# mahfuzalhasan/WaveFormer

Measured on AMD Instinct MI355X. Metric: 128³×4 volumes/sec fwd (1/2/4/8 MI355X) + Dice Δ vs reference, higher is better.
Workload: dtype bf16x3; 1 GPU; MultiscaleTransformer (WaveFormer encoder) forward, 128^3x4 crops; global_batch=8, per_gpu_batch=8, precision=bf16x3, parallelism=replicas x1 (no data-path collective), hip_graph=True

## Files before the change

### waveformer_amd/csrc/ffn_dwfc_tb.hip

```cpp
#include "kernels.hpp"

namespace wf {

#ifndef WF_TB_EPRIO
#define WF_TB_EPRIO 3
#endif

namespace tb4 {
constexpr int S2 = 4;
constexpr int C = 48, HID = 192, TY = 4, TX = 8;
constexpr int PY = TY + 2, PX = TX + 2, PP = PY * PX;
constexpr int NPOS = TY * TX;
constexpr int HS = HID + 8;
constexpr int PLANE_F = PP * HID;
constexpr int H2F = NPOS * HS;
constexpr int NV = HID / 4;
constexpr int NPC = (PP * NV + 63) / 64;
constexpr int NPCE = (NPC + 3) / 4;
constexpr int KS = HID / 32;
constexpr int FWL_BYTES = (C / 16) * KS * 64 * 16;
constexpr size_t LDS_BYTES = (size_t)(2 * PLANE_F + 2 * H2F + 2 * HID + 2 * C) * 4 + FWL_BYTES;
static_assert(LDS_BYTES <= 160 * 1024, "LDS");
}

template <int P>
__global__ __launch_bounds__(1024, 1) void ffn_dwfc_tb4_kernel(DwFcArgs a) {
  using namespace tb4;
  constexpr bool SPLIT = P == PREC_SPLIT;
  __shared__ __attribute__((aligned(16))) float planes[2 * PLANE_F];
  __shared__ __attribute__((aligned(16))) float h2b[2 * H2F];
  __shared__ __attribute__((aligned(16))) float vecs[2 * HID + 2 * C];
  __shared__ bf16x8 fwlo[FWL_BYTES / 16];
  float* lnw = vecs;
  float* lnb = lnw + HID;
  float* fcl = lnb + HID;
  float* n2w = fcl + C;
  __shared__ int simd_cnt[4];

  const int tid = threadIdx.x;
  const int wid = tid >> 6, lane = tid & 63;
  const int D = a.D, H = a.H, W = a.W;
  const int ntx = (W + TX - 1) / TX, nty = (H + TY - 1) / TY, nzs = (D + a.ZS - 1) / a.ZS;
  const int nb = gridDim.x;
  const int xcd = blockIdx.x & 7, q8 = nb >> 3, r8 = nb & 7;
  int t = (xcd < r8 ? xcd * (q8 + 1) : r8 * (q8 + 1) + (xcd - r8) * q8) + (blockIdx.x >> 3);
  const int xt = t % ntx;
  t /= ntx;
  const int yt = t % nty;
  t /= nty;
  const int zt = t % nzs;
  const int b = t / nzs;
  const int x0 = xt * TX, y0 = yt * TY, z0 = zt * a.ZS, z1 = min(z0 + a.ZS, D);
  const int64_t plane_sz = (int64_t)H * W;

  if (tid < 4) simd_cnt[tid] = 0;
  for (int i = tid; i < HID; i += 1024) {
    lnw[i] = 0.5f * a.ln2_w[i];
    lnb[i] = 0.5f * a.ln2_b[i];
  }
  for (int i = tid; i < C; i += 1024) {
    fcl[i] = (a.fc_b ? a.fc_b[i] : 0.f) + (a.stats ? a.n2_b[i] : 0.f);
    n2w[i] = a.stats ? a.n2_w[i] : 1.f;
  }
  if (SPLIT) {
    for (int i = tid; i < (C / 16) * KS * 64; i += 1024) {
      const int l = i & 63, ks = (i >> 6) % KS, ct = (i >> 6) / KS;
      fwlo[i] = *reinterpret_cast<const bf16x8*>(a.fc + (size_t)C * HID +
                                                 (size_t)(ct * 16 + (l & 15)) * HID + ks * 32 + 8 * (l >> 4));
    }
  }
  for (int i = tid; i < HID * 27; i += 1024) planes[i] = a.dw_w[i];
  for (int i = tid; i < HID; i += 1024) planes[HID * 27 + i] = a.dw_b[i];
  __syncthreads();
  const int simd = tb_simd_id();
  int slot = 0;
  if (lane == 0) slot = atomicAdd(&simd_cnt[simd], 1);
  slot = __builtin_amdgcn_readfirstlane(__shfl(slot, 0, 64));
  __syncthreads();
  const bool even = simd_cnt[0] == 4 && simd_cnt[1] == 4 && simd_cnt[2] == 4 && simd_cnt[3] == 4;
  int role = even ? (slot < 3 ? 3 * simd + slot : 12 + simd) : wid;
  role = __builtin_amdgcn_readfirstlane(role);

  if (role < 12) {
    const int cp = role / 3, kslot = role % 3, c = kslot * 64 + lane;
    float w[27];
#pragma unroll
    for (int k = 0; k < 27; ++k) w[k] = planes[c * 27 + k];
    const float bias = planes[HID * 27 + c];
    float acc[3][TY][2];
#pragma unroll
    for (int s = 0; s < 3; ++s)
#pragma unroll
      for (int o = 0; o < TY; ++o) acc[s][o][0] = acc[s][o][1] = 0.f;
    const int lpos = 8 * cp + 4 * kslot + (lane >> 4), lg = lane & 15;
    const int cm = 4 * ((lg - 2 * lpos) & 15);
    __syncthreads();
    __syncthreads();

    auto ln2_rows = [&](float* h2t) {
      constexpr int LNC = HID / 16;
      float* row = h2t + lpos * HS;
      float v[LNC];
#pragma unroll
      for (int j = 0; j < LNC / 4; ++j) {
        const f32x4 u = *reinterpret_cast<const f32x4*>(row + cm + 64 * j);
        v[4 * j] = u.x;
        v[4 * j + 1] = u.y;
        v[4 * j + 2] = u.z;
        v[4 * j + 3] = u.w;
      }
      float s4[4];
#pragma unroll
      for (int j = 0; j < 4; ++j) s4[j] = (v[j] + v[j + 4]) + v[j + 8];
      const float mean = group_sum<16>((s4[0] + s4[1]) + (s4[2] + s4[3])) * (1.f / HID);
      float q4[4];
#pragma unroll
      for (int j = 0; j < 4; ++j) {
        const float d0 = v[j] - mean, d1 = v[j + 4] - mean, d2 = v[j + 8] - mean;
        q4[j] = d2 * d2 + (d1 * d1 + d0 * d0);
      }
      const float rstd = __builtin_amdgcn_rsqf(
          group_sum<16>((q4[0] + q4[1]) + (q4[2] + q4[3])) * (1.f / HID) + a.eps2);
      const float nmr = -mean * rstd;
      uint16_t* rowh = reinterpret_cast<uint16_t*>(row);
#pragma unroll
      for (int j = 0; j < LNC / 4; ++j) {
        const int cc = cm + 64 * j;
        const f32x4 lw4 = *reinterpret_cast<const f32x4*>(lnw + cc);
        const f32x4 lb4 = *reinterpret_cast<const f32x4*>(lnb + cc);
        const f32x4 y = gelu_half4((f32x4{v[4 * j], v[4 * j + 1], v[4 * j + 2], v[4 * j + 3]} *
                                    rstd + nmr) * lw4 + lb4);
        uint32_t h0, h1, l0, l1;
        split_pair<P>(y[0], y[1], h0, l0);
        split_pair<P>(y[2], y[3], h1, l1);
        *reinterpret_cast<u32x2*>(rowh + cc) = u32x2{h0, h1};
        if (SPLIT) *reinterpret_cast<u32x2*>(rowh + HID + cc) = u32x2{l0, l1};
      }
    };
    auto rows = [&](const float (&vin)[PY][4], auto SAc, auto SBc, auto SCc, auto LOc, auto HIc) {
      constexpr int SA = decltype(SAc)::value, SB = decltype(SBc)::value,
                    SC = decltype(SCc)::value, LO = decltype(LOc)::value, HI = decltype(HIc)::value;
#pragma unroll
      for (int r = LO; r < HI; ++r) {
        const float* v = vin[r];
#pragma unroll
        for (int ky = 0; ky < 3; ++ky) {
          const int o = r - ky;
          if (o < 0 || o >= TY) continue;
          const float* w0 = w + ky * 3;
#pragma unroll
          for (int j = 0; j < 2; ++j) {
            if (ky == 0)
              acc[SC][o][j] = w0[2] * v[j + 2] + (w0[1] * v[j + 1] + w0[0] * v[j]);
            else
              acc[SC][o][j] = w0[2] * v[j + 2] + (w0[1] * v[j + 1] + (w0[0] * v[j] + acc[SC][o][j]));
            acc[SB][o][j] = w0[11] * v[j + 2] + (w0[10] * v[j + 1] + (w0[9] * v[j] + acc[SB][o][j]));
            acc[SA][o][j] = w0[20] * v[j + 2] + (w0[19] * v[j + 1] + (w0[18] * v[j] + acc[SA][o][j]));
          }
        }
      }
    };
    typedef std::integral_constant<int, 0> I0;
    typedef std::integral_constant<int, S2> IS;
    typedef std::integral_constant<int, PY> IP;
    auto step = [&](int p, auto Rc) {
      constexpr int R = decltype(Rc)::value;
      typedef std::integral_constant<int, R> SA;
      typedef std::integral_constant<int, (R + 1) % 3> SB;
      typedef std::integral_constant<int, (R + 2) % 3> SC;
      const bool live = p <= z1 && !(ffn_dbg(a) & 1);
      const bool ln = p - 2 >= z0 && p - 2 < z1 && !(ffn_dbg(a) & 2);
      float vin[PY][4];
      const float* q0 = planes + ((p - z0 + 1) & 1) * PLANE_F + 2 * cp * HID + c;
      auto load_plane = [&]() {
#pragma unroll
        for (int r = 0; r < PY; ++r)
#pragma unroll
          for (int k = 0; k < 4; ++k) vin[r][k] = q0[(r * PX + k) * HID];
      };
      if (kslot < 2) {
        if (ln) ln2_rows(h2b + ((p - 2 - z0) & 1) * H2F);
        if (live) load_plane();
      } else if (live) {
        load_plane();
        rows(vin, SA(), SB(), SC(), I0(), IS());
      }
      __syncthreads();
      if (live) {
        if (kslot < 2) rows(vin, SA(), SB(), SC(), I0(), IP());
        else rows(vin, SA(), SB(), SC(), IS(), IP());
        if (p - 1 >= z0) {
          float* h2t = h2b + ((p - 1 - z0) & 1) * H2F;
#pragma unroll
          for (int o = 0; o < TY; ++o)
#pragma unroll
            for (int j = 0; j < 2; ++j)
              h2t[(o * TX + 2 * cp + j) * HS + c] = acc[R][o][j] + bias;
        }
      }
      __syncthreads();
    };
    for (int p = z0 - 1; p <= z1 + 1; p += 3) {
      step(p, std::integral_constant<int, 0>());
      if (p + 1 <= z1 + 1) step(p + 1, std::integral_constant<int, 1>());
      if (p + 2 <= z1 + 1) step(p + 2, std::integral_constant<int, 2>());
    }
    return;
  }

  __builtin_amdgcn_s_setprio(WF_TB_EPRIO);
  const int e = role - 12;
  const int l15 = lane & 15, g4 = lane >> 4;
  const bool has_fc = e < C / 16;
  const int ct = has_fc ? e : 0;
  const float bs = a.bscale ? a.bscale[b] : 1.f;
  bf16x8 fwh[KS];
  {
    const uint16_t* wr = a.fc + (size_t)(ct * 16 + l15) * HID + 8 * g4;
#pragma unroll
    for (int ks = 0; ks < KS; ++ks) fwh[ks] = *reinterpret_cast<const bf16x8*>(wr + ks * 32);
  }
  const bf16x8* fwl = fwlo + ct * KS * 64 + lane;
  const float* src = reinterpret_cast<const float*>(a.h1) + (int64_t)b * D * H * W * HID;
  const int64_t plane_elems = (int64_t)H * W * HID;
  auto piece_off = [&](int k) {
    const int i = min((4 * k + e) * 64 + lane, PP * NV - 1);
    const int pos = i / NV, v = i - pos * NV;
    const int yy = y0 - 1 + pos / PX, xx = x0 - 1 + pos % PX;
    const bool ok = yy >= 0 && yy < H && xx >= 0 && xx < W;
    return ok ? (uint32_t)(((yy * W + xx) * HID + 4 * v) * 4) : 0x80000000u;
  };
  auto stage = [&](int p, float* dst) {
    const bool pz = p >= 0 && p < D;
    const float* base = src + (int64_t)min(max(p, 0), D - 1) * plane_elems;
    const __amdgpu_buffer_rsrc_t rs = __builtin_amdgcn_make_buffer_rsrc(
        const_cast<float*>(base), 0, pz ? (int)(plane_elems * 4) : 0, 0x00020000);
#pragma unroll
    for (int k = 0; k < NPCE; ++k) {
      const int j = 4 * k + e;
      const uint32_t o = piece_off(k);
      if (j * 64 < PP * NV && (j * 64 + lane < PP * NV))
        __builtin_amdgcn_raw_ptr_buffer_load_lds(
            rs, (__attribute__((address_space(3))) void*)(dst + j * 256), 16, o, 0, 0, 0);
    }
  };
  const int col = ct * 16 + 4 * g4;
  const float* sbase = a.stats ? a.stats : a.x;
  auto gpos_of = [&](int zo, int rt, bool clamp) {
    const int lp = rt * 16 + l15;
    int yo = y0 + lp / TX, xo = x0 + lp % TX;
    if (clamp) {
      yo = min(yo, H - 1);
      xo = min(xo, W - 1);
    }
    return (int64_t)b * D * plane_sz + (int64_t)zo * plane_sz + (int64_t)yo * W + xo;
  };
  auto row_ok = [&](int rt) {
    const int lp = rt * 16 + l15;
    return y0 + lp / TX < H && x0 + lp % TX < W;
  };
  f32x4 xr[2][2];
  f32x2 es[2][2];
  const int64_t npos = (int64_t)a.B * D * plane_sz;
  const __amdgpu_buffer_rsrc_t xrsrc = __builtin_amdgcn_make_buffer_rsrc(
      const_cast<float*>(a.x), 0, (int)(npos * C * 4), 0x00020000);
  const __amdgpu_buffer_rsrc_t srsrc = __builtin_amdgcn_make_buffer_rsrc(
      const_cast<float*>(sbase), 0, (int)(npos * 2 * 4), 0x00020000);
  auto load_resid = [&](int zo, f32x4 (&xv)[2], f32x2 (&ev)[2]) {
#pragma unroll
    for (int rt = 0; rt < 2; ++rt) {
      const int g = (int)gpos_of(zo, rt, true);
      xv[rt] = __builtin_bit_cast(f32x4, __builtin_amdgcn_raw_buffer_load_b128(xrsrc, (g * C + col) * 4, 0, 0));
      ev[rt] = __builtin_bit_cast(f32x2, __builtin_amdgcn_raw_buffer_load_b64(srsrc, g * 8, 0, 0));
    }
  };
  const __amdgpu_buffer_rsrc_t orsrc = __builtin_amdgcn_make_buffer_rsrc(
      a.out, 0, (int)(npos * C * 4), 0x00020000);
  auto fc_store = [&](const float* h2t, int zo, int rt, const f32x4& xv, const f32x2& ev) {
    const int lp = rt * 16 + l15;
    f32x4 acc = f32x4{0.f, 0.f, 0.f, 0.f};
    const uint16_t* Bh = reinterpret_cast<const uint16_t*>(h2t) + (size_t)lp * (2 * HS);
#pragma unroll
    for (int ks = 0; ks < KS; ++ks) {
      const int k = ks * 32 + 8 * g4;
      const bf16x8 bh = *reinterpret_cast<const bf16x8*>(Bh + k);
      if (SPLIT) {
        const bf16x8 bl = *reinterpret_cast<const bf16x8*>(Bh + HID + k);
        acc = mma32<P>(fwh[ks], bl, acc);
        acc = mma32<P>(fwl[ks * 64], bh, acc);
      }
      acc = mma32<P>(fwh[ks], bh, acc);
    }
    f32x4 v = acc + *reinterpret_cast<const f32x4*>(fcl + col);
    if (a.stats) {
      const f32x4 lw = *reinterpret_cast<const f32x4*>(n2w + col);
      v = xv + ((xv - ev.x) * ev.y * lw + v) * bs;
    } else {
      v = xv + v * bs;
    }
    const int voff = row_ok(rt) ? (int)((gpos_of(zo, rt, false) * C + col) * 4) : (int)0x80000000;
    __builtin_amdgcn_raw_buffer_store_b128(__builtin_bit_cast(u32x4, v), orsrc, voff, 0, 0);
  };

  __syncthreads();
  stage(z0 - 1, planes);
  asm volatile("s_waitcnt vmcnt(0)" ::: "memory");
  __syncthreads();
  auto iter = [&](int p, auto Sc) {
    constexpr int S = decltype(Sc)::value;
    const int zo = p - 2;
    const bool epi = has_fc && zo >= z0 && zo < z1;
    if (has_fc && zo + 1 >= z0 && zo + 1 < z1) load_resid(zo + 1, xr[S ^ 1], es[S ^ 1]);
    if (p + 1 <= z1 && !(ffn_dbg(a) & 8)) stage(p + 1, planes + ((p + 2 - z0) & 1) * PLANE_F);
    __builtin_amdgcn_s_barrier();
    if (epi && !(ffn_dbg(a) & 4)) {
      const float* h2t = h2b + ((zo - z0) & 1) * H2F;
      fc_store(h2t, zo, 0, xr[S][0], es[S][0]);
      fc_store(h2t, zo, 1, xr[S][1], es[S][1]);
      asm volatile("s_waitcnt vmcnt(2)" ::: "memory");
    } else {
      asm volatile("s_waitcnt vmcnt(0)" ::: "memory");
    }
    asm volatile("s_waitcnt lgkmcnt(0)" ::: "memory");
    __builtin_amdgcn_s_barrier();
  };
  for (int p = z0 - 1; p <= z1 + 1; p += 2) {
    iter(p, std::integral_constant<int, 1>());
    if (p + 1 <= z1 + 1) iter(p + 1, std::integral_constant<int, 0>());
  }
}

int launch_ffn_dwfc_tb4(const DwFcArgs& a, int prec, hipStream_t s) {
  using namespace tb4;
  DwFcArgs g = a;
  static int cus = 0;
  if (!cus) {
    int dev = 0;
    (void)hipGetDevice(&dev);
    (void)hipDeviceGetAttribute(&cus, hipDeviceAttributeMultiprocessorCount, dev);
    if (cus <= 0) cus = 256;
  }
  const int64_t base = (int64_t)g.B * cdiv(g.H, TY) * cdiv(g.W, TX);
  int best_zs = g.D;
  int64_t best = -1;
  for (int nz = 1; nz <= 8 && nz <= g.D; ++nz) {
    const int zs = (int)cdiv(g.D, nz);
    const int64_t cost = cdiv(base * cdiv(g.D, zs), cus) * (zs + 3);
    if (best < 0 || cost < best) {
      best = cost;
      best_zs = zs;
    }
  }
  g.ZS = best_zs;
  g.dbg = ffn_dbg_env();
  const int64_t blocks = base * cdiv(g.D, g.ZS);
  if (prec != PREC_SPLIT && prec != PREC_FP16) return fail(WF_E_SHAPE, "ffn_dwfc_tb4: fp32 h1 only");
  if ((int64_t)g.B * g.D * g.H * g.W * C * 4 >= ((int64_t)1 << 31))
    return fail(WF_E_SHAPE, "ffn_dwfc_tb4: output beyond the 2 GiB buffer-store range");
  void (*kern)(DwFcArgs) = prec == PREC_SPLIT ? ffn_dwfc_tb4_kernel<PREC_SPLIT>
                                              : ffn_dwfc_tb4_kernel<PREC_FP16>;
  hipLaunchKernelGGL(kern, dim3((unsigned)blocks), dim3(1024), 0, s, g);
  return check_launch("ffn_dwfc_tb4");
}

}
```

Baseline: 1237 volumes/s.

## Dedicate one wave to plane prefetch and decouple FC epilogue from loads

```diff
diff --git a/waveformer_amd/csrc/ffn_dwfc_tb.hip b/waveformer_amd/csrc/ffn_dwfc_tb.hip
--- a/waveformer_amd/csrc/ffn_dwfc_tb.hip
+++ b/waveformer_amd/csrc/ffn_dwfc_tb.hip
@@ -1,13 +1,23 @@
 #include "kernels.hpp"
 
 namespace wf {
+
+#ifdef WF_DWFC2_PROBE
+__device__ long long g_dwfctb4_probe[16 * 8];
+extern "C" int wf_debug_dwfctb4_probe(long long* host) {
+  return (int)hipMemcpyFromSymbol(host, HIP_SYMBOL(g_dwfctb4_probe), sizeof(g_dwfctb4_probe));
+}
+#endif
 
 #ifndef WF_TB_EPRIO
 #define WF_TB_EPRIO 3
 #endif
 
 namespace tb4 {
-constexpr int S2 = 4;
+#ifndef WF_TB4_S2
+#define WF_TB4_S2 6
+#endif
+constexpr int S2 = WF_TB4_S2;
 constexpr int C = 48, HID = 192, TY = 4, TX = 8;
 constexpr int PY = TY + 2, PX = TX + 2, PP = PY * PX;
 constexpr int NPOS = TY * TX;
@@ -16,7 +26,12 @@
 constexpr int H2F = NPOS * HS;
 constexpr int NV = HID / 4;
 constexpr int NPC = (PP * NV + 63) / 64;
-constexpr int NPCE = (NPC + 3) / 4;
+static_assert(NPC * 64 == PP * NV, "whole pieces only: the loader issues no partial piece");
+#ifndef WF_TB4_FA
+#define WF_TB4_FA 16
+#endif
+constexpr int FA = WF_TB4_FA;
+static_assert(FA >= 0 && NPC + FA <= 63, "outstanding pieces must fit the 6-bit vmcnt");
 constexpr int KS = HID / 32;
 constexpr int FWL_BYTES = (C / 16) * KS * 64 * 16;
 constexpr size_t LDS_BYTES = (size_t)(2 * PLANE_F + 2 * H2F + 2 * HID + 2 * C) * 4 + FWL_BYTES;
@@ -80,6 +95,11 @@
   const bool even = simd_cnt[0] == 4 && simd_cnt[1] == 4 && simd_cnt[2] == 4 && simd_cnt[3] == 4;
   int role = even ? (slot < 3 ? 3 * simd + slot : 12 + simd) : wid;
   role = __builtin_amdgcn_readfirstlane(role);
+  PROBE_DECL
+#ifdef WF_DWFC2_PROBE
+  pr_acc[6] = role;
+  pr_acc[7] = z1 + 3 - z0;
+#endif
 
   if (role < 12) {
     const int cp = role / 3, kslot = role % 3, c = kslot * 64 + lane;
@@ -185,7 +205,9 @@
         load_plane();
         rows(vin, SA(), SB(), SC(), I0(), IS());
       }
+      PROBE(0)
       __syncthreads();
+      PROBE(1)
       if (live) {
         if (kslot < 2) rows(vin, SA(), SB(), SC(), I0(), IP());
         else rows(vin, SA(), SB(), SC(), IS(), IP());
@@ -198,21 +220,76 @@
               h2t[(o * TX + 2 * cp + j) * HS + c] = acc[R][o][j] + bias;
         }
       }
+      PROBE(2)
       __syncthreads();
+      PROBE(3)
     };
     for (int p = z0 - 1; p <= z1 + 1; p += 3) {
       step(p, std::integral_constant<int, 0>());
       if (p + 1 <= z1 + 1) step(p + 1, std::integral_constant<int, 1>());
       if (p + 2 <= z1 + 1) step(p + 2, std::integral_constant<int, 2>());
     }
+    PROBE_DUMP_TO(g_dwfctb4_probe)
     return;
   }
 
+  const int e = role - 12;
+  if (e == C / 16) {
+    __builtin_amdgcn_s_setprio(3);
+    const float* src = reinterpret_cast<const float*>(a.h1) + (int64_t)b * D * H * W * HID;
+    const int64_t plane_elems = (int64_t)H * W * HID;
+    uint32_t off[NPC];
+#pragma unroll
+    for (int j = 0; j < NPC; ++j) {
+      const int i = j * 64 + lane;
+      const int pos = i / NV, v = i - pos * NV;
+      const int yy = y0 - 1 + pos / PX, xx = x0 - 1 + pos % PX;
+      const bool ok = yy >= 0 && yy < H && xx >= 0 && xx < W;
+      off[j] = ok ? (uint32_t)(((yy * W + xx) * HID + 4 * v) * 4) : 0x80000000u;
+    }
+    auto fill = [&](int p, auto LOc, auto HIc) {
+      constexpr int LO = decltype(LOc)::value, HI = decltype(HIc)::value;
+      float* dst = planes + ((p - z0 + 1) & 1) * PLANE_F;
+      const bool pz = p >= 0 && p < D;
+      const float* base = src + (int64_t)min(max(p, 0), D - 1) * plane_elems;
+      const __amdgpu_buffer_rsrc_t rs = __builtin_amdgcn_make_buffer_rsrc(
+          const_cast<float*>(base), 0, pz ? (int)(plane_elems * 4) : 0, 0x00020000);
+#pragma unroll
+      for (int j = LO; j < HI; ++j)
+        __builtin_amdgcn_raw_ptr_buffer_load_lds(
+            rs, (__attribute__((address_space(3))) void*)(dst + j * 256), 16, off[j], 0, 0, 0);
+    };
+    typedef std::integral_constant<int, 0> F0;
+    typedef std::integral_constant<int, FA> FAc;
+    typedef std::integral_constant<int, NPC> FN;
+    const bool fetch = !(ffn_dbg(a) & 8);
+    __syncthreads();
+    fill(z0 - 1, F0(), FN());
+    fill(z0, F0(), FAc());
+    asm volatile("s_waitcnt vmcnt(%0)" ::"n"(FA) : "memory");
+    __builtin_amdgcn_s_barrier();
+    for (int p = z0 - 1; p <= z1 + 1; ++p) {
+      if (p + 1 <= z1 && fetch) fill(p + 1, FAc(), FN());
+      PROBE(4)
+      __builtin_amdgcn_s_barrier();
+      PROBE(1)
+      if (p + 2 <= z1 && fetch) {
+        fill(p + 2, F0(), FAc());
+        PROBE(2)
+        asm volatile("s_waitcnt vmcnt(%0)" ::"n"(FA) : "memory");
+      } else {
+        asm volatile("s_waitcnt vmcnt(0)" ::: "memory");
+      }
+      PROBE(5)
+      __builtin_amdgcn_s_barrier();
+      PROBE(3)
+    }
+    PROBE_DUMP_TO(g_dwfctb4_probe)
+    return;
+  }
   __builtin_amdgcn_s_setprio(WF_TB_EPRIO);
-  const int e = role - 12;
   const int l15 = lane & 15, g4 = lane >> 4;
-  const bool has_fc = e < C / 16;
-  const int ct = has_fc ? e : 0;
+  const int ct = e;
   const float bs = a.bscale ? a.bscale[b] : 1.f;
   bf16x8 fwh[KS];
   {
@@ -221,29 +298,6 @@
     for (int ks = 0; ks < KS; ++ks) fwh[ks] = *reinterpret_cast<const bf16x8*>(wr + ks * 32);
   }
   const bf16x8* fwl = fwlo + ct * KS * 64 + lane;
-  const float* src = reinterpret_cast<const float*>(a.h1) + (int64_t)b * D * H * W * HID;
-  const int64_t plane_elems = (int64_t)H * W * HID;
-  auto piece_off = [&](int k) {
-    const int i = min((4 * k + e) * 64 + lane, PP * NV - 1);
-    const int pos = i / NV, v = i - pos * NV;
-    const int yy = y0 - 1 + pos / PX, xx = x0 - 1 + pos % PX;
-    const bool ok = yy >= 0 && yy < H && xx >= 0 && xx < W;
-    return ok ? (uint32_t)(((yy * W + xx) * HID + 4 * v) * 4) : 0x80000000u;
-  };
-  auto stage = [&](int p, float* dst) {
-    const bool pz = p >= 0 && p < D;
-    const float* base = src + (int64_t)min(max(p, 0), D - 1) * plane_elems;
-    const __amdgpu_buffer_rsrc_t rs = __builtin_amdgcn_make_buffer_rsrc(
-        const_cast<float*>(base), 0, pz ? (int)(plane_elems * 4) : 0, 0x00020000);
-#pragma unroll
-    for (int k = 0; k < NPCE; ++k) {
-      const int j = 4 * k + e;
-      const uint32_t o = piece_off(k);
-      if (j * 64 < PP * NV && (j * 64 + lane < PP * NV))
-        __builtin_amdgcn_raw_ptr_buffer_load_lds(
-            rs, (__attribute__((address_space(3))) void*)(dst + j * 256), 16, o, 0, 0, 0);
-    }
-  };
   const int col = ct * 16 + 4 * g4;
   const float* sbase = a.stats ? a.stats : a.x;
   auto gpos_of = [&](int zo, int rt, bool clamp) {
@@ -303,31 +357,35 @@
   };
 
   __syncthreads();
-  stage(z0 - 1, planes);
-  asm volatile("s_waitcnt vmcnt(0)" ::: "memory");
   __syncthreads();
-  auto iter = [&](int p, auto Sc) {
+  auto fc_tile = [&](int zo, auto Sc) {
     constexpr int S = decltype(Sc)::value;
-    const int zo = p - 2;
-    const bool epi = has_fc && zo >= z0 && zo < z1;
-    if (has_fc && zo + 1 >= z0 && zo + 1 < z1) load_resid(zo + 1, xr[S ^ 1], es[S ^ 1]);
-    if (p + 1 <= z1 && !(ffn_dbg(a) & 8)) stage(p + 1, planes + ((p + 2 - z0) & 1) * PLANE_F);
-    __builtin_amdgcn_s_barrier();
-    if (epi && !(ffn_dbg(a) & 4)) {
+    if (zo >= z0 && zo < z1 && !(ffn_dbg(a) & 4)) {
       const float* h2t = h2b + ((zo - z0) & 1) * H2F;
       fc_store(h2t, zo, 0, xr[S][0], es[S][0]);
       fc_store(h2t, zo, 1, xr[S][1], es[S][1]);
-      asm volatile("s_waitcnt vmcnt(2)" ::: "memory");
-    } else {
-      asm volatile("s_waitcnt vmcnt(0)" ::: "memory");
-    }
+    }
+  };
+  auto iter = [&](int p, auto Sc) {
+    constexpr int S = decltype(Sc)::value;
+    const int zo = p - 3;
+    fc_tile(zo, Sc);
+    PROBE(2)
+    if (zo + 1 >= z0 && zo + 1 < z1) load_resid(zo + 1, xr[S ^ 1], es[S ^ 1]);
+    PROBE(0)
     asm volatile("s_waitcnt lgkmcnt(0)" ::: "memory");
     __builtin_amdgcn_s_barrier();
+    PROBE(1)
+    __builtin_amdgcn_s_barrier();
+    PROBE(3)
   };
   for (int p = z0 - 1; p <= z1 + 1; p += 2) {
-    iter(p, std::integral_constant<int, 1>());
-    if (p + 1 <= z1 + 1) iter(p + 1, std::integral_constant<int, 0>());
-  }
+    iter(p, std::integral_constant<int, 0>());
+    if (p + 1 <= z1 + 1) iter(p + 1, std::integral_constant<int, 1>());
+  }
+  if ((z1 - 1 - z0) & 1) fc_tile(z1 - 1, std::integral_constant<int, 1>());
+  else fc_tile(z1 - 1, std::integral_constant<int, 0>());
+  PROBE_DUMP_TO(g_dwfctb4_probe)
 }
 
 int launch_ffn_dwfc_tb4(const DwFcArgs& a, int prec, hipStream_t s) {
```

Result: faster. 1292 volumes/s (median of 6 runs) (+4.5%).
